# Shadowfear36/SegHiero

Hardware: AMD Instinct MI355X
Metric: images/sec at 512x512 (ResNet-50 2-level), full train step (higher is better)
Workload: dtype f32 (convolutions: exact 3-way bf16 split of every fp32 operand, 6 bf16 MFMA products, f32 accumulate; rest plain f32)

## Files before the change

seghiero_amd/csrc/conv_x6p.hip:

```cpp
#include "conv_x6.h"

__device__ __forceinline__ int swz_row(int row) { return ((row >> 2) & 3) ^ (row & 2); }

#ifndef SH_W1
#define SH_W1(AFF, EPI) ((AFF) == 2 ? 2 : 3)
#define SH_W2(AFF, EPI) (((AFF) == 2 || (EPI) == 2) ? 3 : 4)
#endif
#ifndef SH_X6P_PART
#define SH_X6P_PART 0
#endif
#define SH_PART(n) (SH_X6P_PART == 0 || SH_X6P_PART == (n))
int sh_x6p_launch_dgrad(ConvQ& p, hipStream_t st, int force);
int sh_x6p_wgrad_l0b0(ConvQ& p, bool aff, int wgm, int wgn, int splits, hipStream_t st);
int sh_x6p_wgrad_l1b0(ConvQ& p, bool aff, int wgm, int wgn, int splits, hipStream_t st);
int sh_x6p_wgrad_l0b1(ConvQ& p, bool aff, int wgm, int wgn, int splits, hipStream_t st);
int sh_x6p_wgrad_l1b1(ConvQ& p, bool aff, int wgm, int wgn, int splits, hipStream_t st);
static int x6p_mode() { static int v = -2; if (v == -2) { const char* e = getenv("SEGHIERO_X6P"); v = e ? atoi(e) : 1; } return v; }
[[maybe_unused]] static int x6p_ws() { static int v = -2; if (v == -2) { const char* e = getenv("SEGHIERO_X6P_WS"); v = e ? atoi(e) : 0; } return v; }
static int x6p_tile() { static int v = -2; if (v == -2) { const char* e = getenv("SEGHIERO_X6P_TILE"); v = e ? atoi(e) : 0; } return v; }
#if SH_PART(1) || SH_PART(2) || defined(SH_X6P_EXP)
template <int MODE, int TM, int TN, int WGM, int WGN, int WPS, int AFF, int EPI, int SK, int TAP, int GRP = 0, int ABF = 0, int WS = 0>
__global__ __launch_bounds__(64 * WGM * WGN * (WS ? 2 : 1), WPS) void conv_x6p_kernel(const ConvQ p) {
    constexpr int NT = 64 * WGM * WGN;
    constexpr int BM = 32 * TM * WGM, BN = 32 * TN * WGN;
    constexpr int A_PLANE = BM * ROWB, B_PLANE = BN * ROWB;
    constexpr int RPP = NT / 4;
    constexpr int NA = BM / RPP, NB = BN / RPP;
    static_assert(BM % RPP == 0 && BN % RPP == 0 && RPP % 64 == 0, "tile / thread-count mismatch");
    extern __shared__ __attribute__((aligned(16))) unsigned char smem[];
    unsigned char* const As = smem;
    unsigned char* const Bs = smem + 3 * A_PLANE;
    float* const coef = reinterpret_cast<float*>(smem + 3 * (A_PLANE + B_PLANE));
    static_assert(AFF != 2 || (MODE == DGRAD && TAP == 0 && !GRP), "the deferred BatchNorm-backward loader exists for 1x1 dgrads");
    static_assert(!ABF || (MODE == FPROP && !GRP) || AFF == 2, "bf16 loader streams: the fprop input, or the y stream of the lin loader");
    constexpr bool A_BF = ABF && MODE == FPROP, A2_BF = ABF && AFF == 2;
    constexpr bool A3 = A_BF && AFF == 0;
    auto load_a4 = [&](const __amdgpu_buffer_rsrc_t& rs, unsigned elem_off, unsigned ok, bool bf) -> f32x4 {
        if (bf) {
            const unsigned voff = ((elem_off * 2u) & ok) | (0x80000000u & ~ok);
            const u32x2 r = __builtin_bit_cast(u32x2, __builtin_amdgcn_raw_buffer_load_b64(rs, voff, 0, 0));
            return f32x4{__uint_as_float(r[0]), __uint_as_float(r[1]), 0.f, 0.f};
        }
        const unsigned voff = ((elem_off * 4u) & ok) | (0x80000000u & ~ok);
        return __builtin_bit_cast(f32x4, __builtin_amdgcn_raw_buffer_load_b128(rs, voff, 0, 0));
    };
    auto widen_a4 = [&](f32x4 v, bool bf) -> f32x4 {
        return bf ? bf16x4_to_f32(sh_u32x2{__float_as_uint(v[0]), __float_as_uint(v[1])}) : v;
    };

    const int t_all = threadIdx.x, t = WS ? (t_all & (NT - 1)) : t_all, lane = t & 63, wave = t >> 6;
    [[maybe_unused]] const bool producer = WS && t_all >= NT;
    static_assert(!WS || (NT & (NT - 1)) == 0, "wave-specialised form: power-of-two wave count");
    const int wm = wave / WGN, wn = wave % WGN, l31 = lane & 31, h = lane >> 5;
    const unsigned nblk = (unsigned)p.tiles_m * (unsigned)p.tiles_n;
    const unsigned bid = xcd_remap(blockIdx.x, nblk);
    const int tile_n = bid % p.tiles_n, tile_m = bid / p.tiles_n;
    const int m0 = tile_m * BM, n0 = tile_n * BN;
    const int grp = GRP ? n0 / p.group_n : 0;
    const float* const a_ptr = GRP ? p.ga[grp] : p.a;
    const float* const b_ptr = GRP ? p.gb[grp] : p.b;
    const unsigned a_bytes = GRP ? p.ga_bytes[grp] : p.a_bytes;
    const int lda = (int)(GRP ? p.glda[grp] : p.lda);
    const float* const sc_ptr = GRP ? p.gsc[grp] : p.aff_scale;
    const float* const sh_ptr = GRP ? p.gsh[grp] : p.aff_shift;
    const float aff_floor = (GRP && sc_ptr == nullptr) ? -INFINITY : 0.f;
    int cy = 0, cx = 0, Hc = p.H, Wc = p.W, oy0 = 0, ox0 = 0, ntw = p.KW, Mc = p.M, Kt = p.K;
    if constexpr (MODE == DGRAD) {
        if (p.parity) {
            cy = blockIdx.y >> 1; cx = blockIdx.y & 1;
            oy0 = (cy + p.pad) & 1; ox0 = (cx + p.pad) & 1;
            Hc = (p.H - oy0 + 1) >> 1; Wc = (p.W - ox0 + 1) >> 1;
            const int nth = (p.KH - cy + 1) >> 1;
            ntw = (p.KW - cx + 1) >> 1;
            Mc = p.N * Hc * Wc; Kt = nth * ntw * p.Kc;
            if (m0 >= Mc) return;
        }
    }
    int q_begin = 0, q_end = (Kt + 15) >> 4;
    if constexpr (SK) {
        const int per = ((q_end + p.ksplit - 1) / p.ksplit + 1) & ~1;
        q_begin = min(q_end, (int)blockIdx.y * per); q_end = min(q_end, q_begin + per);
    }
    const int klim = min(Kt, 16 * q_end);
    const int nq = (q_end - q_begin + 1) & ~1;
    constexpr bool single_tap = TAP == 0, tap_uniform = TAP <= 1;

    const __amdgpu_buffer_rsrc_t rsrc_a = __builtin_amdgcn_make_buffer_rsrc(const_cast<float*>(a_ptr), 0, a_bytes, 0x00020000);
    const __amdgpu_buffer_rsrc_t rsrc_b = __builtin_amdgcn_make_buffer_rsrc(const_cast<float*>(b_ptr), 0, p.b_bytes, 0x00020000);
    [[maybe_unused]] const __amdgpu_buffer_rsrc_t rsrc_a2 =
        __builtin_amdgcn_make_buffer_rsrc(const_cast<float*>(AFF == 2 ? p.a2 : a_ptr), 0, AFF == 2 ? p.a2_bytes : a_bytes, 0x00020000);
    constexpr unsigned OOB = 0x80000000u;
    const int kc = t & 3, r0 = t >> 2;
    int a_y[NA], a_x[NA], a_nb[NA];
    int b_row[NB];
    unsigned b_ok[NB];
    int cur_tap = -1;
    const bool direct = TAP == 0 && p.stride == 1 && p.pad == 0 && !(MODE == DGRAD && (p.parity || p.scatter));
#pragma unroll
    for (int i = 0; i < NA; ++i) {
        const int m = m0 + r0 + RPP * i;
        if (direct) { a_y[i] = m < Mc ? 0 : -(1 << 28); a_x[i] = 0; a_nb[i] = m < Mc ? m : 0; }
        else if (m < Mc) {
            if constexpr (MODE == FPROP) {
                const int ow = m % p.Wo, q = m / p.Wo, oh = q % p.Ho, n = q / p.Ho;
                a_y[i] = oh * p.stride - p.pad; a_x[i] = ow * p.stride - p.pad; a_nb[i] = n * p.H * p.W;
            } else {
                const int iwc = m % Wc, q = m / Wc, ihc = q % Hc, n = q / Hc;
                const int ih = p.parity ? 2 * ihc + oy0 : ihc, iw = p.parity ? 2 * iwc + ox0 : iwc;
                a_y[i] = ih + p.pad; a_x[i] = iw + p.pad; a_nb[i] = n * p.Ho * p.Wo;
            }
        } else { a_y[i] = -(1 << 28); a_x[i] = 0; a_nb[i] = 0; }
    }
#pragma unroll
    for (int i = 0; i < NB; ++i) {
        const int j = n0 + r0 + RPP * i;
        b_ok[i] = j < p.Nn ? ~0u : 0u;
        b_row[i] = (GRP ? j - grp * p.group_n : j) * (MODE == FPROP ? p.K : p.Kc);
    }
    int a_off[NA];
    [[maybe_unused]] int a_off2[NA];
    unsigned a_ok[NA];
    auto set_tap = [&](int tap) {
        if (direct) {
#pragma unroll
            for (int i = 0; i < NA; ++i) {
                a_ok[i] = a_y[i] == 0 ? ~0u : 0u;
                a_off[i] = a_nb[i] * lda;
                if constexpr (AFF == 2) a_off2[i] = a_nb[i] * (int)p.lda2;
            }
            return;
        }
        int kh, kw;
        if (MODE == DGRAD && p.parity) { const int ty = tap / ntw; kh = cy + 2 * ty; kw = cx + 2 * (tap - ty * ntw); }
        else { kh = tap / p.KW; kw = tap - kh * p.KW; }
        const int dh = kh * p.dil, dw = kw * p.dil;
#pragma unroll
        for (int i = 0; i < NA; ++i) {
            if constexpr (MODE == FPROP) {
                const int ih = a_y[i] + dh, iw = a_x[i] + dw;
                a_ok[i] = ((unsigned)ih < (unsigned)p.H && (unsigned)iw < (unsigned)p.W) ? ~0u : 0u;
                a_off[i] = (a_nb[i] + ih * p.W + iw) * lda;
            } else {
                int th = a_y[i] - dh, tw = a_x[i] - dw;
                bool ok = th >= 0 && tw >= 0;
                if (p.stride > 1) {
                    ok = ok && (th % p.stride == 0) && (tw % p.stride == 0);
                    th /= p.stride; tw /= p.stride;
                }
                a_ok[i] = (ok && th < p.Ho && tw < p.Wo) ? ~0u : 0u;
                a_off[i] = (a_nb[i] + th * p.Wo + tw) * lda;
                if constexpr (AFF == 2) a_off2[i] = (a_nb[i] + th * p.Wo + tw) * (int)p.lda2;
            }
        }
    };
    auto prepare_tap = [&](int q) {
        if constexpr (TAP == 1) {
            const int tap = (16 * q) / p.Kc;
            if (tap != cur_tap) { set_tap(tap); cur_tap = tap; }
        }
    };
    if constexpr (TAP == 0) { set_tap(0); cur_tap = 0; }
    const f32x4 zero4 = {0.f, 0.f, 0.f, 0.f};
    struct Regs { f32x4 a[NA]; f32x4 a2[AFF == 2 ? NA : 1]; f32x4 b[NB]; int cc; unsigned okm; };
    auto load_half = [&](int q, Regs& R) {
        const int kbase = 16 * q, k = kbase + 4 * kc;
        int tap, cc;
        if constexpr (single_tap) { tap = 0; cc = k; }
        else if constexpr (tap_uniform) { tap = cur_tap; cc = k - tap * p.Kc; }
        else { tap = k / p.Kc; cc = k - tap * p.Kc; set_tap(tap); }
        const unsigned kok = (unsigned)((k - klim) >> 31);
        int wtap = tap;
        if (MODE == DGRAD && p.parity) { const int ty = tap / ntw; wtap = (cy + 2 * ty) * p.KW + cx + 2 * (tap - ty * ntw); }
        R.cc = cc; R.okm = 0;
#pragma unroll
        for (int i = 0; i < NA; ++i) {
            const unsigned ok = kok & a_ok[i];
            R.a[i] = load_a4(rsrc_a, (unsigned)(a_off[i] + cc), ok, A_BF);
            if constexpr (AFF == 2) R.a2[i] = load_a4(rsrc_a2, (unsigned)(a_off2[i] + cc), ok, A2_BF);
            if (AFF) R.okm |= ok & (1u << i);
        }
#pragma unroll
        for (int i = 0; i < NB; ++i) {
            int off;
            if constexpr (MODE == FPROP) off = b_row[i] + k;
            else off = wtap * p.Cin * p.Kc + b_row[i] + cc;
            const unsigned okb = kok & b_ok[i];
            const unsigned voff = (((unsigned)off * 4u) & okb) | (OOB & ~okb);
            R.b[i] = __builtin_bit_cast(f32x4, __builtin_amdgcn_raw_buffer_load_b128(rsrc_b, voff, 0, 0));
        }
    };
    const int swz_w = swz_row(r0);
    auto store_half = [&](Regs& R, int hb) {
        const int off0 = r0 * ROWB + ((((2 * hb) | (kc >> 1)) ^ swz_w) << 4) + ((kc & 1) << 3);
        f32x4 sc = zero4, sh = zero4;
        [[maybe_unused]] f32x4 lmu = zero4, ld_ = zero4;
        if constexpr (AFF) { sc = *reinterpret_cast<const f32x4*>(coef + R.cc); sh = *reinterpret_cast<const f32x4*>(coef + p.Kc + R.cc); }
        if constexpr (AFF == 2) { lmu = *reinterpret_cast<const f32x4*>(coef + 2 * p.Kc + R.cc); ld_ = *reinterpret_cast<const f32x4*>(coef + 3 * p.Kc + R.cc); }
#pragma unroll
        for (int i = 0; i < NA; ++i) {
            if constexpr (A3) {
                *reinterpret_cast<u32x2*>(As + off0 + RPP * i * ROWB) = u32x2{__float_as_uint(R.a[i][0]), __float_as_uint(R.a[i][1])};
                continue;
            }
            f32x4 v = widen_a4(R.a[i], A_BF);
            if constexpr (AFF == 2) {
                const bool ok = (R.okm >> i) & 1u;
                const f32x4 y2 = widen_a4(R.a2[i], A2_BF);
#pragma unroll
                for (int e = 0; e < 4; ++e) { const float w = fmaf(y2[e] - lmu[e], sh[e], fmaf(v[e], sc[e], ld_[e])); v[e] = ok ? w : 0.f; }
            } else if constexpr (AFF) {
                const bool ok = (R.okm >> i) & 1u;
#pragma unroll
                for (int e = 0; e < 4; ++e) { const float w = fmaxf(v[e] * sc[e] + sh[e], aff_floor); v[e] = ok ? w : 0.f; }
            }
            u32x2 q1, q2, q3;
            split4(v, q1, q2, q3);
            const int off = off0 + RPP * i * ROWB;
            *reinterpret_cast<u32x2*>(As + off) = q1;
            *reinterpret_cast<u32x2*>(As + A_PLANE + off) = q2;
            *reinterpret_cast<u32x2*>(As + 2 * A_PLANE + off) = q3;
        }
#pragma unroll
        for (int i = 0; i < NB; ++i) {
            u32x2 q1, q2, q3;
#ifdef SH_ABLATE_BSPLIT
            q1[0] = __float_as_uint(R.b[i][0]); q1[1] = __float_as_uint(R.b[i][1]); q2 = q1; q3[0] = __float_as_uint(R.b[i][2]); q3[1] = __float_as_uint(R.b[i][3]);
#else
            split4(R.b[i], q1, q2, q3);
#endif
            const int off = off0 + RPP * i * ROWB;
            *reinterpret_cast<u32x2*>(Bs + off) = q1;
            *reinterpret_cast<u32x2*>(Bs + B_PLANE + off) = q2;
            *reinterpret_cast<u32x2*>(Bs + 2 * B_PLANE + off) = q3;
        }
    };

    f32x16 acc[TM][TN];
#pragma unroll
    for (int i = 0; i < TM; ++i)
#pragma unroll
        for (int j = 0; j < TN; ++j)
#pragma unroll
            for (int r = 0; r < 16; ++r) acc[i][j][r] = 0.f;

    const int arow = wm * 32 * TM + l31, brow = wn * 32 * TN + l31;
    const int swz_r = swz_row(l31);
    auto compute_half = [&](int hb) {
        const int rd = (((2 * hb) | h) ^ swz_r) << 4;
        bf16x8 bfr[TN][3];
#pragma unroll
        for (int j = 0; j < TN; ++j)
#pragma unroll
            for (int pl = 0; pl < 3; ++pl)
                bfr[j][pl] = __builtin_bit_cast(bf16x8, *reinterpret_cast<const u32x4*>(Bs + pl * B_PLANE + (brow + 32 * j) * ROWB + rd));
#pragma unroll
        for (int i = 0; i < TM; ++i) {
            if constexpr (A3) {
                const bf16x8 a0 = __builtin_bit_cast(bf16x8, *reinterpret_cast<const u32x4*>(As + (arow + 32 * i) * ROWB + rd));
#pragma unroll
                for (int j = 0; j < TN; ++j) acc[i][j] = mma3(a0, bfr[j], acc[i][j]);
            } else {
            bf16x8 af[3];
#pragma unroll
            for (int pl = 0; pl < 3; ++pl)
                af[pl] = __builtin_bit_cast(bf16x8, *reinterpret_cast<const u32x4*>(As + pl * A_PLANE + (arow + 32 * i) * ROWB + rd));
#pragma unroll
            for (int j = 0; j < TN; ++j) acc[i][j] = mma6(af, bfr[j], acc[i][j]);
            }
        }
    };

    auto phase_schedule = [&]() {
        constexpr int PA = A3 ? 1 : 3, PP = A3 ? 3 : 6;
        constexpr int NMFMA = TM * TN * PP, NVALU = 30 * ((A3 ? 0 : NA) + NB) + (AFF == 2 ? 16 : 8 * AFF) * NA, NDSW = PA * NA + 3 * NB,
                      NVM = NA + NB + (AFF == 2 ? NA : 0);
        constexpr int VPM = (NVALU + NMFMA - 1) / NMFMA;
        __builtin_amdgcn_sched_group_barrier(0x100, 3 * TN + PA, 0);
#pragma unroll
        for (int g = 0; g < NMFMA; ++g) {
            __builtin_amdgcn_sched_group_barrier(0x008, 1, 0);
            __builtin_amdgcn_sched_group_barrier(0x002, VPM, 0);
            if (g * NDSW / NMFMA != (g + 1) * NDSW / NMFMA) __builtin_amdgcn_sched_group_barrier(0x200, 1, 0);
            if (g * NVM / NMFMA != (g + 1) * NVM / NMFMA) __builtin_amdgcn_sched_group_barrier(0x020, 1, 0);
            if (g % (PP * TN) == 2 && g / (PP * TN) + 1 < TM) __builtin_amdgcn_sched_group_barrier(0x100, PA, 0);
        }
    };
    if constexpr (AFF == 2) {
        for (int c = t_all; c < 4 * p.Kc; c += NT * (WS ? 2 : 1)) coef[c] = p.lin[c];
        __syncthreads();
    } else if constexpr (AFF) {
        for (int c = t_all; c < p.Kc; c += NT * (WS ? 2 : 1)) { coef[c] = sc_ptr ? sc_ptr[c] : 1.f; coef[p.Kc + c] = sh_ptr ? sh_ptr[c] : 0.f; }
        __syncthreads();
    }
    if constexpr (WS) {
        if (producer) {
            Regs R0, R1;
            prepare_tap(q_begin);     load_half(q_begin, R0);
            prepare_tap(q_begin + 1); load_half(q_begin + 1, R1);
            store_half(R0, 0);
            prepare_tap(q_begin + 2); load_half(q_begin + 2, R0);
            __syncthreads();
            for (int j = 0; j < nq; j += 2) {
                prepare_tap(q_begin + j + 3);
                store_half(R1, 1);
                load_half(q_begin + j + 3, R1);
                __syncthreads();
                prepare_tap(q_begin + j + 4);
                store_half(R0, 0);
                load_half(q_begin + j + 4, R0);
                __syncthreads();
            }
            return;
        }
        __syncthreads();
        for (int j = 0; j < nq; j += 2) {
            compute_half(0);
            __syncthreads();
            compute_half(1);
            __syncthreads();
        }
    } else {
    Regs R0, R1;
    prepare_tap(q_begin);     load_half(q_begin, R0);
    prepare_tap(q_begin + 1); load_half(q_begin + 1, R1);
    store_half(R0, 0);
    prepare_tap(q_begin + 2); load_half(q_begin + 2, R0);
    __syncthreads();
    for (int j = 0; j < nq; j += 2) {
        prepare_tap(q_begin + j + 3);
        store_half(R1, 1);
        load_half(q_begin + j + 3, R1);
        compute_half(0);
        phase_schedule();
        __syncthreads();
        prepare_tap(q_begin + j + 4);
        store_half(R0, 0);
        load_half(q_begin + j + 4, R0);
        compute_half(1);
        phase_schedule();
        __syncthreads();
    }
    }

    if constexpr (SK) {
        float* slab = p.slab + (long long)blockIdx.y * p.M * p.ldslab;
#pragma unroll
        for (int j = 0; j < TN; ++j) {
            const int n = n0 + wn * 32 * TN + 32 * j + l31;
#pragma unroll
            for (int i = 0; i < TM; ++i)
#pragma unroll
                for (int r = 0; r < 16; ++r) {
                    const int m = m0 + wm * 32 * TM + 32 * i + (r & 3) + 8 * (r >> 2) + 4 * h;
                    if (m < p.M && n < p.Nn) slab[(long long)m * p.ldslab + n] = acc[i][j][r];
                }
        }
        return;
    }

    static_assert(EPI == 0 || TM % 2 == 0, "statistics epilogues need whole 64-row groups per wave");
    int ncol[TN];
    bool nok[TN];
    float bias[TN];
    [[maybe_unused]] float b_mu[TN], b_is[TN], b_sc[TN], b_sh[TN];
#pragma unroll
    for (int j = 0; j < TN; ++j) {
        ncol[j] = n0 + wn * 32 * TN + 32 * j + l31;
        nok[j] = ncol[j] < p.Nn;
        bias[j] = (MODE == FPROP && p.extra != nullptr && nok[j]) ? p.extra[ncol[j]] : 0.f;
        if constexpr (EPI == 2) {
            b_mu[j] = b_is[j] = b_sc[j] = b_sh[j] = 0.f;
            if (nok[j]) { b_mu[j] = p.bnb_mean[ncol[j]]; b_is[j] = p.bnb_invstd[ncol[j]]; b_sc[j] = p.bnb_scale[ncol[j]]; b_sh[j] = p.bnb_shift[ncol[j]]; }
        }
    }
    if (EPI == 2 || p.vec_epi) {
        constexpr int WC = 32 * TN, RS = WC + 4, LPR = WC / 4, RPI = 64 / LPR, NRD = 32 / RPI;
        float* const stage = reinterpret_cast<float*>(smem) + wave * (32 * RS);
        const int rr = lane / LPR, c4 = (lane % LPR) * 4;
        const int ncv = n0 + wn * WC + c4;
        const bool nokv = ncv < p.Nn;
        f32x4 vb = zero4, v_mu = zero4, v_is = zero4, v_sc = zero4, v_sh = zero4;
        if (MODE == FPROP && p.extra != nullptr && nokv) vb = ld4(p.extra + ncv);
        if constexpr (EPI == 2) { if (nokv) { v_mu = ld4(p.bnb_mean + ncv); v_is = ld4(p.bnb_invstd + ncv); v_sc = ld4(p.bnb_scale + ncv); v_sh = ld4(p.bnb_shift + ncv); } }
        [[maybe_unused]] f32x4 pend_gs = zero4, pend_gq = zero4;
#pragma unroll
        for (int i = 0; i < TM; ++i) {
#pragma unroll
            for (int j = 0; j < TN; ++j)
#pragma unroll
                for (int r = 0; r < 16; ++r) stage[((r & 3) + 8 * (r >> 2) + 4 * h) * RS + 32 * j + l31] = acc[i][j][r];
            constexpr int CH = (EPI == 2 && NRD > 4) ? 4 : NRD;
            [[maybe_unused]] f32x4 gs = zero4, gq = zero4;
#pragma unroll
            for (int k0 = 0; k0 < NRD; k0 += CH) {
            f32x4 v[CH];
            [[maybe_unused]] f32x4 ad[CH], yv[CH], ov[CH];
            long long mrow[CH];
#pragma unroll
            for (int kk = 0; kk < CH; ++kk) {
                const int row = (k0 + kk) * RPI + rr;
                mrow[kk] = m0 + wm * 32 * TM + 32 * i + row;
                v[kk] = *reinterpret_cast<const f32x4*>(stage + row * RS + c4);
                if constexpr (MODE == DGRAD) {
                    ad[kk] = zero4;
                    if (mrow[kk] < Mc && nokv) {
                        if (p.extra != nullptr) ad[kk] = ld4(p.extra + mrow[kk] * p.ldadd + ncv);
                        if constexpr (EPI == 2) {
                            yv[kk] = lda4(p.bnb_y, mrow[kk] * p.bnb_ldy + ncv, p.act & 4);
                            if (p.bnb_out != nullptr)
                                ov[kk] = (p.act & 64) ? quad_mask_load(p.bnb_out, mrow[kk] * p.bnb_ldo + (ncv >> 2)) : lda4(p.bnb_out, mrow[kk] * p.bnb_ldo + ncv, p.act & 8);
                        }
                    }
                }
            }
#pragma unroll
            for (int kk = 0; kk < CH; ++kk) {
                if (mrow[kk] < Mc && nokv) {
                    f32x4 o = v[kk];
                    if constexpr (MODE == FPROP) o += vb;
                    else {
                        o += ad[kk];
                        if constexpr (EPI == 2) {
                            if (p.bnb_relu) {
                                const f32x4 a = p.bnb_out != nullptr ? ov[kk] : yv[kk] * v_sc + v_sh;
#pragma unroll
                                for (int e = 0; e < 4; ++e) if (!(a[e] > 0.f)) o[e] = 0.f;
                            }
                            gs += o; gq += o * ((yv[kk] - v_mu) * v_is);
                        }
                    }
                    sta4(p.c, mrow[kk] * p.ldc + ncv, o, MODE == FPROP ? (p.act & 2) : 0);
                }
            }
            }
            if constexpr (EPI == 2) {
#pragma unroll
                for (int e = 0; e < 4; ++e) {
#pragma unroll
                    for (int o2 = LPR; o2 < 64; o2 <<= 1) { gs[e] += __shfl_xor(gs[e], o2, 64); gq[e] += __shfl_xor(gq[e], o2, 64); }
                }
                if ((i & 1) == 0) { pend_gs = gs; pend_gq = gq; }
                else {
                    const int pidx = tile_m * (BM / 64) + wm * (TM / 2) + (i >> 1);
                    if (lane < LPR && pidx < p.n_partials && nokv) {
                        st4(p.partials + ((long long)pidx * 2 + 0) * p.Nn + ncv, pend_gs + gs);
                        st4(p.partials + ((long long)pidx * 2 + 1) * p.Nn + ncv, pend_gq + gq);
                    }
                }
            }
        }
    } else if constexpr (EPI != 2) {
    [[maybe_unused]] float pend_s[TN], pend_q[TN];
#pragma unroll
    for (int i = 0; i < TM; ++i) {
        [[maybe_unused]] float gs[TN], gq[TN];
#pragma unroll
        for (int j = 0; j < TN; ++j) { gs[j] = 0.f; gq[j] = 0.f; }
        long long orow[16];
        bool mok[16];
        [[maybe_unused]] float ad[16][TN], yv[16][TN];
#pragma unroll
        for (int r = 0; r < 16; ++r) {
            const int m = m0 + wm * 32 * TM + 32 * i + (r & 3) + 8 * (r >> 2) + 4 * h;
            mok[r] = m < Mc;
            orow[r] = m;
            if constexpr (MODE == DGRAD) {
                if (p.parity) {
                    const int iwc = m % Wc, q2 = m / Wc, ihc = q2 % Hc, nb2 = q2 / Hc;
                    orow[r] = ((long long)nb2 * p.H + 2 * ihc + oy0) * p.W + 2 * iwc + ox0;
                } else if (p.scatter) {
                    const int ow = m % p.W, q = m / p.W, oh = q % p.H, nb = q / p.H;
                    orow[r] = (long long)(nb * p.sH + oh * p.sstride) * p.sW + ow * p.sstride;
                }
#pragma unroll
                for (int j = 0; j < TN; ++j) {
                    ad[r][j] = 0.f;
                    if (mok[r] && nok[j]) {
                        if (p.scatter) ad[r][j] = p.c[orow[r] * p.ldc + ncol[j]];
                        else if (p.extra != nullptr) ad[r][j] = p.extra[orow[r] * p.ldadd + ncol[j]];
                        if constexpr (EPI == 2) yv[r][j] = p.bnb_y[orow[r] * p.bnb_ldy + ncol[j]];
                    }
                }
            }
        }
#pragma unroll
        for (int r = 0; r < 16; ++r) {
#pragma unroll
            for (int j = 0; j < TN; ++j) {
                if (mok[r] && nok[j]) {
                    float v = acc[i][j][r];
                    float* dst = p.c + orow[r] * p.ldc + ncol[j];
                    if constexpr (MODE == FPROP) {
                        *dst = v + bias[j];
                    } else {
                        v += ad[r][j];
                        if constexpr (EPI == 2) {
                            if (p.bnb_relu && !(yv[r][j] * b_sc[j] + b_sh[j] > 0.f)) v = 0.f;
                            gs[j] += v; gq[j] += v * ((yv[r][j] - b_mu[j]) * b_is[j]);
                        }
                        *dst = v;
                    }
                }
            }
        }
        if constexpr (EPI == 2) {
#pragma unroll
            for (int j = 0; j < TN; ++j) {
                const float s1 = gs[j] + __shfl_xor(gs[j], 32, 64), q1 = gq[j] + __shfl_xor(gq[j], 32, 64);
                if ((i & 1) == 0) { pend_s[j] = s1; pend_q[j] = q1; }
                else {
                    const int pidx = tile_m * (BM / 64) + wm * (TM / 2) + (i >> 1);
                    if (h == 0 && pidx < p.n_partials && nok[j]) {
                        p.partials[((long long)pidx * 2 + 0) * p.Nn + ncol[j]] = pend_s[j] + s1;
                        p.partials[((long long)pidx * 2 + 1) * p.Nn + ncol[j]] = pend_q[j] + q1;
                    }
                }
            }
        }
    }
    }
    if constexpr (MODE == FPROP && EPI == 1) {
        if (p.partials != nullptr) {
            const int wrow0 = m0 + wm * 32 * TM;
#pragma unroll
            for (int pr = 0; pr < TM / 2; ++pr) {
                const int prow0 = wrow0 + 64 * pr;
                const int npr = max(0, min(64, p.M - prow0));
                const int pidx = tile_m * (BM / 64) + wm * (TM / 2) + pr;
#pragma unroll
                for (int j = 0; j < TN; ++j) {
                    float ss = 0.f;
#pragma unroll
                    for (int i = 2 * pr; i < 2 * pr + 2; ++i)
#pragma unroll
                        for (int r = 0; r < 16; ++r) ss += acc[i][j][r];
                    ss += __shfl_xor(ss, 32, 64);
                    const float mean = npr > 0 ? ss / (float)npr : 0.f;
                    float qq = 0.f;
#pragma unroll
                    for (int i = 2 * pr; i < 2 * pr + 2; ++i)
#pragma unroll
                        for (int r = 0; r < 16; ++r) {
                            const int row = wrow0 + 32 * i + (r & 3) + 8 * (r >> 2) + 4 * h;
                            const float dv = acc[i][j][r] - mean;
                            qq += (npr == 64 || row < p.M) ? dv * dv : 0.f;
                        }
                    qq += __shfl_xor(qq, 32, 64);
                    const int n = n0 + wn * 32 * TN + 32 * j + l31;
                    if (h == 0 && pidx < p.n_partials && n < p.Nn) {
                        p.partials[((long long)pidx * 2 + 0) * p.Nn + n] = ss;
                        p.partials[((long long)pidx * 2 + 1) * p.Nn + n] = qq;
                    }
                }
            }
        }
    }
}

template <int MODE, int TM, int TN, int WGM, int WGN, int WPS, int AFF, int EPI, int SK, int TAP, int GRP = 0, int ABF = 0, int WS = 0>
static int launch_x6p(ConvQ& p, hipStream_t st) {
    constexpr int BM = 32 * TM * WGM, BN = 32 * TN * WGN;
    const size_t lds = 3 * (size_t)(BM + BN) * ROWB + (AFF == 2 ? 16 : AFF ? 8 : 0) * (size_t)p.Kc;
    if (lds > 160 * 1024) return SH_X6P_NO;
    static size_t attr_lds = 0;
    if (lds > attr_lds) {
        (void)hipFuncSetAttribute(reinterpret_cast<const void*>(&conv_x6p_kernel<MODE, TM, TN, WGM, WGN, WPS, AFF, EPI, SK, TAP, GRP, ABF, WS>),
                                  hipFuncAttributeMaxDynamicSharedMemorySize, (int)(160 * 1024));
        attr_lds = 160 * 1024;
    }
    p.tiles_m = (int)sh_cdiv(p.M, BM);
    p.tiles_n = (int)sh_cdiv(p.Nn, BN);
    dim3 grid((unsigned)(p.tiles_m * p.tiles_n), p.parity ? 4u : (SK ? (unsigned)p.ksplit : 1u));
    conv_x6p_kernel<MODE, TM, TN, WGM, WGN, WPS, AFF, EPI, SK, TAP, GRP, ABF, WS><<<grid, 64 * WGM * WGN * (WS ? 2 : 1), lds, st>>>(p);
    return sh_launch_status();
}

template <int MODE, int AFF, int EPI, int TAP, int ABF = 0>
static int pick_tile_x6p(ConvQ& p, hipStream_t st, int force) {
    (void)force;
    constexpr int W1 = SH_W1(AFF, EPI), W2 = SH_W2(AFF, EPI);
#ifdef SH_X6P_WS
    if (p.Nn > 64 && x6p_ws()) return launch_x6p<MODE, 2, 2, 2, 2, 2, AFF, EPI, 0, TAP, 0, ABF, 1>(p, st);
#endif
    if (p.Nn > 64) return launch_x6p<MODE, 2, 2, 2, 2, W1, AFF, EPI, 0, TAP, 0, ABF>(p, st);
    return launch_x6p<MODE, 2, 1, 2, 2, W2, AFF, EPI, 0, TAP, 0, ABF>(p, st);
}

template <int MODE, int AFF, int EPI, int ABF = 0>
static int pick_x6p(ConvQ& p, hipStream_t st, int force) {
    if constexpr (AFF == 2) {
        if (p.KH * p.KW != 1) return SH_X6P_NO;
        if (p.ksplit > 1) {
            const int rc = launch_x6p<MODE, 2, 2, 2, 2, 2, 2, 0, 1, 0, 0, ABF>(p, st);
            return rc == SH_OK ? sh_x6_splitk_reduce(p, MODE, st) : rc;
        }
        return pick_tile_x6p<MODE, 2, EPI, 0, ABF>(p, st, force);
    } else {
    if (p.ksplit > 1) {
        int rc;
        if (p.KH * p.KW == 1) rc = launch_x6p<MODE, 2, 2, 2, 2, 3, AFF, 0, 1, 0, 0, ABF>(p, st);
        else if ((p.Kc & 15) == 0) rc = launch_x6p<MODE, 2, 2, 2, 2, 3, AFF, 0, 1, 1, 0, ABF>(p, st);
        else return SH_X6P_NO;
        return rc == SH_OK ? sh_x6_splitk_reduce(p, MODE, st) : rc;
    }
    if (p.KH * p.KW == 1) return pick_tile_x6p<MODE, AFF, EPI, 0, ABF>(p, st, force);
    if ((p.Kc & 15) == 0) return pick_tile_x6p<MODE, AFF, EPI, 1, ABF>(p, st, force);
    if (AFF || EPI == 2 || ABF) return SH_X6P_NO;
    return pick_tile_x6p<MODE, 0, EPI, 2>(p, st, force);
    }
}

#endif
#if SH_PART(1)

int sh_x6p_grouped_launch(ConvQ& p, hipStream_t st) {
    if (p.ngroups < 1 || p.ngroups > 6 || (p.group_n & 127) || p.KH * p.KW != 1) return SH_X6P_NO;
    auto al16 = [](const void* q) { return ((uintptr_t)q & 15) == 0; };
    p.vec_epi = (p.ldc & 3) == 0 && al16(p.c);
    return launch_x6p<FPROP, 2, 2, 2, 2, 3, 1, 1, 0, 0, 1>(p, st);
}

int sh_x6p_launch(int mode, ConvQ& p, hipStream_t st) {
    const bool aff = p.aff_scale != nullptr, bnb = p.bnb_y != nullptr;
    if (!x6p_mode() && !aff && !bnb && !p.lin) return SH_X6P_NO;
    const int force = x6p_tile();
    auto al16 = [](const void* q) { return ((uintptr_t)q & 15) == 0; };
    p.vec_epi = !p.parity && !p.scatter && (p.Nn & 3) == 0 && (p.ldc & 3) == 0 && al16(p.c) &&
                (p.extra == nullptr || (al16(p.extra) && (mode == FPROP || (p.ldadd & 3) == 0))) &&
                (!bnb || ((p.bnb_ldy & 3) == 0 && al16(p.bnb_y) && (p.bnb_out == nullptr || (p.act & 64) || ((p.bnb_ldo & 3) == 0 && al16(p.bnb_out))) && al16(p.bnb_mean) && al16(p.bnb_invstd) && al16(p.bnb_scale) &&
                          al16(p.bnb_shift) && al16(p.partials)));
    if (bnb && !p.vec_epi) return SH_X6P_NO;
    { static int v = -2; if (v == -2) { const char* e = getenv("SEGHIERO_X6P_VEC"); v = e ? atoi(e) : 1; } if (!v && !bnb) p.vec_epi = 0; }
    if ((p.act & 2) && !p.vec_epi) return SH_X6P_NO;
    if (mode == FPROP) {
        if (bnb) return SH_EINVAL;
        if (p.act & 1) return aff ? pick_x6p<FPROP, 1, 1, 1>(p, st, force) : pick_x6p<FPROP, 0, 1, 1>(p, st, force);
        if (aff) return pick_x6p<FPROP, 1, 1>(p, st, force);
        return pick_x6p<FPROP, 0, 1>(p, st, force);
    }
    if (aff) return SH_EINVAL;
    return sh_x6p_launch_dgrad(p, st, force);
}
#endif
#if SH_PART(2)
int sh_x6p_launch_dgrad(ConvQ& p, hipStream_t st, int force) {
    const bool bnb = p.bnb_y != nullptr;
    if (p.lin != nullptr && (p.act & 16)) return bnb ? pick_x6p<DGRAD, 2, 2, 1>(p, st, force) : pick_x6p<DGRAD, 2, 0, 1>(p, st, force);
    if (p.lin != nullptr) return bnb ? pick_x6p<DGRAD, 2, 2>(p, st, force) : pick_x6p<DGRAD, 2, 0>(p, st, force);
    if (bnb) return pick_x6p<DGRAD, 0, 2>(p, st, force);
    return pick_x6p<DGRAD, 0, 0>(p, st, force);
}
#endif

#if SH_X6P_PART == 0 || SH_X6P_PART >= 3
template <int WGM, int WGN, int AFF, int LIN = 0, int XBF = 0>
__global__ __launch_bounds__(64 * WGM * WGN, 2) void conv_wgrad_x6p_kernel(const ConvQ p) {
    constexpr int NT = 64 * WGM * WGN, BM = 64 * WGM, BN = 64 * WGN;
    constexpr bool X3 = XBF && AFF == 0;
    constexpr int AROWB = 2 * BM + 64, BROWB = 2 * BN + 64;
    constexpr int APLANE = 32 * AROWB, BPLANE = 32 * BROWB;
    constexpr int ACPR = BM / 4, BCPR = BN / 4;
    constexpr int AKPP = NT / ACPR, BKPP = NT / BCPR;
    constexpr int NA = 16 / AKPP, NB = 16 / BKPP;
    static_assert(NA >= 1 && NB >= 1, "a loader pass must not straddle the two halves");
    extern __shared__ __attribute__((aligned(16))) unsigned char smem[];
    unsigned char* const As = smem;
    unsigned char* const Bs = smem + 3 * APLANE;
    const int t = threadIdx.x, lane = t & 63, wave = t >> 6;
    const int wm = wave / WGN, wn = wave % WGN, l31 = lane & 31, h = lane >> 5;
    const unsigned nblk = (unsigned)p.tiles_m * (unsigned)p.tiles_n;
    unsigned slice, bid;
    if (p.scatter) { const unsigned kq = blockIdx.x >> 3; slice = (kq / nblk) * 8u + (blockIdx.x & 7u); bid = kq % nblk; }
    else { slice = blockIdx.x / nblk; bid = xcd_remap(blockIdx.x % nblk, nblk); }
    if (slice >= (unsigned)p.ksplit) return;
    const int tile_n = bid % p.tiles_n, tile_m = bid / p.tiles_n;
    const int m0 = tile_m * BM, n0 = tile_n * BN;
    const int kbeg = slice * p.kchunk, kend = min(p.K, kbeg + p.kchunk);
    const int nq = (((kend - kbeg + 15) >> 4) + 1) & ~1;

    const __amdgpu_buffer_rsrc_t rsrc_a = __builtin_amdgcn_make_buffer_rsrc(const_cast<float*>(p.a), 0, p.a_bytes, 0x00020000);
    const __amdgpu_buffer_rsrc_t rsrc_b = __builtin_amdgcn_make_buffer_rsrc(const_cast<float*>(p.b), 0, p.b_bytes, 0x00020000);
    [[maybe_unused]] const __amdgpu_buffer_rsrc_t rsrc_a2 =
        __builtin_amdgcn_make_buffer_rsrc(const_cast<float*>(LIN ? p.a2 : p.a), 0, LIN ? p.a2_bytes : p.a_bytes, 0x00020000);
    constexpr unsigned OOB = 0x80000000u;
    const int arc = t % ACPR, ak0 = t / ACPR;
    const int brc = t % BCPR, bk0 = t / BCPR;
    const int co = m0 + 4 * arc;
    const int nn = n0 + 4 * brc;
    const unsigned a_col_ok = co < p.M ? ~0u : 0u, b_col_ok = nn < p.Nn ? ~0u : 0u;
    const int tap = nn / p.Cin, wg_ci = nn - tap * p.Cin;
    const int kh = tap / p.KW, kw = tap - kh * p.KW;
    const int wg_dh = kh * p.dil - p.pad, wg_dw = kw * p.dil - p.pad;
    f32x4 sc = {0.f, 0.f, 0.f, 0.f}, sh = sc;
    if constexpr (AFF) { if (b_col_ok) { sc = ld4(p.aff_scale + wg_ci); sh = ld4(p.aff_shift + wg_ci); } }
    [[maybe_unused]] f32x4 lA = sc, lB = sc, lM = sc, lD = sc;
    if constexpr (LIN) { lA = lB = lM = lD = f32x4{0.f, 0.f, 0.f, 0.f}; if (a_col_ok) { lA = ld4(p.lin + co); lB = ld4(p.lin + p.M + co); lM = ld4(p.lin + 2 * p.M + co); lD = ld4(p.lin + 3 * p.M + co); } }
    int px_ow[NB], px_oh[NB], px_n[NB];
#pragma unroll
    for (int i = 0; i < NB; ++i) {
        const int pix = kbeg + bk0 + BKPP * i;
        px_ow[i] = pix % p.Wo; const int q2 = pix / p.Wo; px_oh[i] = q2 % p.Ho; px_n[i] = q2 / p.Ho;
    }
    auto wg_load4 = [&](const __amdgpu_buffer_rsrc_t& rs, unsigned elem_off, unsigned ok, bool bf) -> f32x4 {
        if (bf) {
            const unsigned voff = ((elem_off * 2u) & ok) | (OOB & ~ok);
            const u32x2 r = __builtin_bit_cast(u32x2, __builtin_amdgcn_raw_buffer_load_b64(rs, voff, 0, 0));
            return f32x4{__uint_as_float(r[0]), __uint_as_float(r[1]), 0.f, 0.f};
        }
        const unsigned voff = ((elem_off * 4u) & ok) | (OOB & ~ok);
        return __builtin_bit_cast(f32x4, __builtin_amdgcn_raw_buffer_load_b128(rs, voff, 0, 0));
    };
    auto wg_widen = [&](f32x4 v, bool bf) -> f32x4 { return bf ? bf16x4_to_f32(sh_u32x2{__float_as_uint(v[0]), __float_as_uint(v[1])}) : v; };
    struct Regs { f32x4 a[NA]; f32x4 a2[LIN ? NA : 1]; f32x4 b[NB]; unsigned okm, okl; };
    auto load_half = [&](int q, Regs& R) {
        const int kbase = kbeg + 16 * q;
        R.okm = 0; R.okl = 0;
#pragma unroll
        for (int i = 0; i < NA; ++i) {
            const int pix = kbase + ak0 + AKPP * i;
            const unsigned ok = (unsigned)((pix - kend) >> 31) & a_col_ok;
            const unsigned voff = (((unsigned)(pix * (int)p.lda + co) * 4u) & ok) | (OOB & ~ok);
            R.a[i] = __builtin_bit_cast(f32x4, __builtin_amdgcn_raw_buffer_load_b128(rsrc_a, voff, 0, 0));
            if constexpr (LIN) {
                R.a2[i] = wg_load4(rsrc_a2, (unsigned)(pix * (int)p.lda2 + co), ok, XBF);
                R.okl |= ok & (1u << i);
            }
        }
#pragma unroll
        for (int i = 0; i < NB; ++i) {
            const int pix = kbase + bk0 + BKPP * i;
            const int ih = px_oh[i] * p.stride + wg_dh, iw = px_ow[i] * p.stride + wg_dw;
            const unsigned inimg = ((unsigned)ih < (unsigned)p.H && (unsigned)iw < (unsigned)p.W) ? ~0u : 0u;
            const unsigned ok = (unsigned)((pix - kend) >> 31) & b_col_ok & inimg;
            R.b[i] = wg_load4(rsrc_b, (unsigned)(((px_n[i] * p.H + ih) * p.W + iw) * (int)p.ldb + wg_ci), ok, XBF);
            if (AFF) R.okm |= ok & (1u << i);
            int ow = px_ow[i] + 16, oh = px_oh[i], n = px_n[i];
            const bool c1 = ow >= p.Wo; ow -= c1 ? p.Wo : 0; oh += c1 ? 1 : 0;
            const bool c2 = oh >= p.Ho; oh -= c2 ? p.Ho : 0; n += c2 ? 1 : 0;
            px_ow[i] = ow; px_oh[i] = oh; px_n[i] = n;
        }
    };
    auto store_half = [&](Regs& R, int hb) {
#pragma unroll
        for (int i = 0; i < NA; ++i) {
            const int off = (16 * hb + ak0 + AKPP * i) * AROWB + arc * 8;
            u32x2 q1, q2, q3;
            f32x4 va = R.a[i];
            if constexpr (LIN) {
                const bool ok = (R.okl >> i) & 1u;
                const f32x4 y2 = wg_widen(R.a2[i], XBF);
#pragma unroll
                for (int e = 0; e < 4; ++e) { const float w = fmaf(y2[e] - lM[e], lB[e], fmaf(va[e], lA[e], lD[e])); va[e] = ok ? w : 0.f; }
            }
            split4(va, q1, q2, q3);
            *reinterpret_cast<u32x2*>(As + off) = q1;
            *reinterpret_cast<u32x2*>(As + APLANE + off) = q2;
            *reinterpret_cast<u32x2*>(As + 2 * APLANE + off) = q3;
        }
#pragma unroll
        for (int i = 0; i < NB; ++i) {
            if constexpr (X3) {
                *reinterpret_cast<u32x2*>(Bs + (16 * hb + bk0 + BKPP * i) * BROWB + brc * 8) = u32x2{__float_as_uint(R.b[i][0]), __float_as_uint(R.b[i][1])};
                continue;
            }
            f32x4 v = wg_widen(R.b[i], XBF);
            if constexpr (AFF) {
                const bool ok = (R.okm >> i) & 1u;
#pragma unroll
                for (int e = 0; e < 4; ++e) { const float w = fmaxf(v[e] * sc[e] + sh[e], 0.f); v[e] = ok ? w : 0.f; }
            }
            const int off = (16 * hb + bk0 + BKPP * i) * BROWB + brc * 8;
            u32x2 q1, q2, q3;
            split4(v, q1, q2, q3);
            *reinterpret_cast<u32x2*>(Bs + off) = q1;
            *reinterpret_cast<u32x2*>(Bs + BPLANE + off) = q2;
            *reinterpret_cast<u32x2*>(Bs + 2 * BPLANE + off) = q3;
        }
    };
    f32x16 acc[2][2];
#pragma unroll
    for (int i = 0; i < 2; ++i)
#pragma unroll
        for (int j = 0; j < 2; ++j)
#pragma unroll
            for (int r = 0; r < 16; ++r) acc[i][j][r] = 0.f;
    const int g = lane >> 4, li = lane & 15, qq = li >> 2, pp = li & 3;
    const int krow = (g >> 1) * 8 + qq, coff = (16 * (g & 1) + 4 * pp) * 2;
    auto frag = [&](const unsigned char* plane, int rowb, int hb, int rowbase) -> bf16x8 {
        const unsigned char* a0 = plane + (krow + hb * 16) * rowb + coff + rowbase * 2;
        const s16x4 v0 = __builtin_amdgcn_ds_read_tr16_b64_v4i16((s16x4 __attribute__((address_space(3)))*)(a0));
        const s16x4 v1 = __builtin_amdgcn_ds_read_tr16_b64_v4i16((s16x4 __attribute__((address_space(3)))*)(a0 + 4 * rowb));
        s16x8 r;
        r[0] = v0[0]; r[1] = v0[1]; r[2] = v0[2]; r[3] = v0[3]; r[4] = v1[0]; r[5] = v1[1]; r[6] = v1[2]; r[7] = v1[3];
        return __builtin_bit_cast(bf16x8, r);
    };
    auto compute_half = [&](int hb) {
        bf16x8 af[2][3], bfr[2][X3 ? 1 : 3];
#pragma unroll
        for (int i = 0; i < 2; ++i)
#pragma unroll
            for (int pl = 0; pl < 3; ++pl) {
                af[i][pl] = frag(As + pl * APLANE, AROWB, hb, wm * 64 + 32 * i);
                if (!X3 || pl == 0) bfr[i][X3 ? 0 : pl] = frag(Bs + pl * BPLANE, BROWB, hb, wn * 64 + 32 * i);
            }
#pragma unroll
        for (int i = 0; i < 2; ++i)
#pragma unroll
            for (int j = 0; j < 2; ++j) {
                if constexpr (X3) acc[i][j] = mma3b(af[i], bfr[j][0], acc[i][j]);
                else acc[i][j] = mma6(af[i], bfr[j], acc[i][j]);
            }
    };
    auto phase_schedule = [&]() {
        constexpr int NMF = X3 ? 12 : 24, NDSR = X3 ? 8 : 12;
        constexpr int NVALU = (X3 ? 2 : 30 + 8 * AFF) * NB + (30 + 16 * LIN) * NA + 8 * NB, NDSW = 3 * NA + (X3 ? 1 : 3) * NB, NVM = NA + NB + LIN * NA;
        constexpr int VPM = (NVALU + NMF - 1) / NMF;
        __builtin_amdgcn_sched_group_barrier(0x100, NDSR, 0);
#pragma unroll
        for (int gq = 0; gq < NMF; ++gq) {
            __builtin_amdgcn_sched_group_barrier(0x008, 1, 0);
            __builtin_amdgcn_sched_group_barrier(0x002, VPM, 0);
            if (gq * NDSW / NMF != (gq + 1) * NDSW / NMF) __builtin_amdgcn_sched_group_barrier(0x200, 1, 0);
            if (gq * NVM / NMF != (gq + 1) * NVM / NMF) __builtin_amdgcn_sched_group_barrier(0x020, 1, 0);
            if (gq == 2) __builtin_amdgcn_sched_group_barrier(0x100, NDSR, 0);
        }
    };
    Regs R0, R1;
    load_half(0, R0);
    load_half(1, R1);
    store_half(R0, 0);
    load_half(2, R0);
    __syncthreads();
    for (int j = 0; j < nq; j += 2) {
        store_half(R1, 1);
        load_half(j + 3, R1);
        compute_half(0);
        phase_schedule();
        __syncthreads();
        store_half(R0, 0);
        load_half(j + 4, R0);
        compute_half(1);
        phase_schedule();
        __syncthreads();
    }
    float* slab = p.c + (long long)slice * p.M * p.Nn;
#pragma unroll
    for (int i = 0; i < 2; ++i)
#pragma unroll
        for (int j = 0; j < 2; ++j) {
            const int n = n0 + wn * 64 + 32 * j + l31;
#pragma unroll
            for (int r = 0; r < 16; ++r) {
                const int m = m0 + wm * 64 + 32 * i + (r & 3) + 8 * (r >> 2) + 4 * h;
                if (m < p.M && n < p.Nn) slab[(long long)m * p.Nn + n] = acc[i][j][r];
            }
        }
}
template <int WGM, int WGN, int AFF, int LIN = 0, int XBF = 0>
static int launch_wgrad_x6p(ConvQ& p, int splits, hipStream_t st) {
    constexpr size_t lds = 3 * 32 * (size_t)((2 * 64 * WGM + 64) + (2 * 64 * WGN + 64));
    static bool attr_done = false;
    if (!attr_done) {
        (void)hipFuncSetAttribute(reinterpret_cast<const void*>(&conv_wgrad_x6p_kernel<WGM, WGN, AFF, LIN, XBF>), hipFuncAttributeMaxDynamicSharedMemorySize, (int)lds);
        attr_done = true;
    }
    p.tiles_m = (int)sh_cdiv(p.M, 64 * WGM); p.tiles_n = (int)sh_cdiv(p.Nn, 64 * WGN);
    p.ksplit = splits;
    const unsigned grid = (unsigned)(p.tiles_m * p.tiles_n) * (unsigned)(p.scatter ? sh_cdiv(splits, 8) * 8 : splits);
    conv_wgrad_x6p_kernel<WGM, WGN, AFF, LIN, XBF><<<grid, 64 * WGM * WGN, lds, st>>>(p);
    return sh_launch_status();
}
template <int AFF, int LIN = 0, int XBF = 0>
static int pick_wgrad_x6p(ConvQ& p, int wgm, int wgn, int splits, hipStream_t st) {
    if (wgm == 4 && wgn == 1) return launch_wgrad_x6p<4, 1, AFF, LIN, XBF>(p, splits, st);
    if (wgm == 2 && wgn == 1) return launch_wgrad_x6p<2, 1, AFF, LIN, XBF>(p, splits, st);
    if (wgm == 2 && wgn == 4) return launch_wgrad_x6p<2, 4, AFF, LIN, XBF>(p, splits, st);
    if (wgm == 1 && wgn == 4) return launch_wgrad_x6p<1, 4, AFF, LIN, XBF>(p, splits, st);
    if (wgm == 1 && wgn == 2) return launch_wgrad_x6p<1, 2, AFF, LIN, XBF>(p, splits, st);
    return launch_wgrad_x6p<2, 2, AFF, LIN, XBF>(p, splits, st);
}
#if SH_PART(3)
int sh_x6p_wgrad_l0b0(ConvQ& p, bool aff, int wgm, int wgn, int splits, hipStream_t st) {
    return aff ? pick_wgrad_x6p<1>(p, wgm, wgn, splits, st) : pick_wgrad_x6p<0>(p, wgm, wgn, splits, st);
}
int sh_x6p_wgrad_launch(ConvQ& p, int wgm, int wgn, int splits, hipStream_t st) {
    const bool aff = p.aff_scale != nullptr;
    if (!x6p_mode() && !aff && !p.lin) return SH_X6P_NO;
    if (p.Wo < 16 || (p.Cin & 3)) return SH_X6P_NO;
    if (p.act & 32) {
        if (p.lin != nullptr && !(p.act & 16)) return SH_X6P_NO;
        return p.lin != nullptr ? sh_x6p_wgrad_l1b1(p, aff, wgm, wgn, splits, st) : sh_x6p_wgrad_l0b1(p, aff, wgm, wgn, splits, st);
    }
    if (p.lin != nullptr && (p.act & 16)) return SH_X6P_NO;
    return p.lin != nullptr ? sh_x6p_wgrad_l1b0(p, aff, wgm, wgn, splits, st) : sh_x6p_wgrad_l0b0(p, aff, wgm, wgn, splits, st);
}
#endif
#if SH_PART(4)
int sh_x6p_wgrad_l1b0(ConvQ& p, bool aff, int wgm, int wgn, int splits, hipStream_t st) {
    return aff ? pick_wgrad_x6p<1, 1>(p, wgm, wgn, splits, st) : pick_wgrad_x6p<0, 1>(p, wgm, wgn, splits, st);
}
#endif
#if SH_PART(5)
int sh_x6p_wgrad_l0b1(ConvQ& p, bool aff, int wgm, int wgn, int splits, hipStream_t st) {
    return aff ? pick_wgrad_x6p<1, 0, 1>(p, wgm, wgn, splits, st) : pick_wgrad_x6p<0, 0, 1>(p, wgm, wgn, splits, st);
}
#endif
#if SH_PART(6)
int sh_x6p_wgrad_l1b1(ConvQ& p, bool aff, int wgm, int wgn, int splits, hipStream_t st) {
    return aff ? pick_wgrad_x6p<1, 1, 1>(p, wgm, wgn, splits, st) : pick_wgrad_x6p<0, 1, 1>(p, wgm, wgn, splits, st);
}
#endif
#endif

#ifdef SH_X6P_EXP
template __global__ void conv_x6p_kernel<SH_X6P_EXP>(const ConvQ);
#endif
```

Measured before the change: 501.3.

## Prefetch BatchNorm-backward epilogue inputs during the dgrad main loop

Adds a dedicated epilogue path for the fused BatchNorm-backward dgrad kernel. It issues the buffer loads of the forward activation y and the ReLU mask a few iterations before the main K loop ends, so their latency overlaps with MFMA work. It also loads the residual-add strips one row group ahead inside the epilogue. The occupancy hints for EPI==2 are lowered to 2 waves per SIMD to make room for the extra prefetch registers, with a fallback to 3 for very large grids. The costs are higher register pressure and lower occupancy, which could hurt the main loop.

```diff
diff --git a/seghiero_amd/csrc/conv_x6p.hip b/seghiero_amd/csrc/conv_x6p.hip
--- a/seghiero_amd/csrc/conv_x6p.hip
+++ b/seghiero_amd/csrc/conv_x6p.hip
@@ -3,9 +3,11 @@
 __device__ __forceinline__ int swz_row(int row) { return ((row >> 2) & 3) ^ (row & 2); }
 
 #ifndef SH_W1
-#define SH_W1(AFF, EPI) ((AFF) == 2 ? 2 : 3)
-#define SH_W2(AFF, EPI) (((AFF) == 2 || (EPI) == 2) ? 3 : 4)
-#endif
+#define SH_W1(AFF, EPI) (((AFF) == 2 || (EPI) == 2) ? 2 : 3)
+#define SH_W2(AFF, EPI) ((EPI) == 2 ? 2 : (AFF) == 2 ? 3 : 4)
+#endif
+#define SH_BNB_PRE_TILES 4096
+#define SH_BNB_LEAD 4
 #ifndef SH_X6P_PART
 #define SH_X6P_PART 0
 #endif
@@ -285,6 +287,57 @@
             if (g % (PP * TN) == 2 && g / (PP * TN) + 1 < TM) __builtin_amdgcn_sched_group_barrier(0x100, PA, 0);
         }
     };
+    constexpr bool PRE = EPI == 2 && WPS <= 2 && (AFF != 2 || TN == 1);
+    static_assert(!PRE || (MODE == DGRAD && !SK && !WS), "the BatchNorm-backward epilogue belongs to the one-pass dgrad");
+    constexpr int E_WC = 32 * TN, E_LPR = E_WC / 4, E_RPI = 64 / E_LPR, E_NRD = 32 / E_RPI;
+    [[maybe_unused]] auto e_pos = [&](int& rr, int& cc) {
+        int tt = t;
+        asm volatile("" : "+v"(tt));
+        const int ln = tt & 63, wv = tt >> 6;
+        rr = (wv / WGN) * 32 * TM + ln / E_LPR; cc = (wv % WGN) * E_WC + (ln % E_LPR) * 4;
+    };
+    constexpr bool E_QM = AFF != 2;
+    [[maybe_unused]] f32x4 ypre[PRE ? TM : 1][PRE ? E_NRD : 1];
+    [[maybe_unused]] unsigned mpre[PRE ? E_NRD : 1];
+    [[maybe_unused]] auto prefetch_bnb = [&]() {
+        int e_rr, e_cc;
+        e_pos(e_rr, e_cc);
+        auto e_ok = [&](int i, int k) -> unsigned { return (m0 + e_rr + 32 * i + k * E_RPI < Mc && n0 + e_cc < p.Nn) ? ~0u : 0u; };
+        const int ybf = (p.act & 4) ? 1 : 0;
+        const __amdgpu_buffer_rsrc_t rs_y = __builtin_amdgcn_make_buffer_rsrc(
+            const_cast<char*>(reinterpret_cast<const char*>(p.bnb_y)) + ((long long)m0 * p.bnb_ldy + n0) * (ybf ? 2 : 4), 0, OOB, 0x00020000);
+        const int ldy = (int)p.bnb_ldy;
+        if (ybf) {
+#pragma unroll
+            for (int i = 0; i < (PRE ? TM : 0); ++i)
+#pragma unroll
+                for (int k = 0; k < E_NRD; ++k) {
+                    const unsigned ok = e_ok(i, k);
+                    const unsigned voff = ((unsigned)(((e_rr + 32 * i + k * E_RPI) * ldy + e_cc) * 2) & ok) | (OOB & ~ok);
+                    const u32x2 r = __builtin_bit_cast(u32x2, __builtin_amdgcn_raw_buffer_load_b64(rs_y, voff, 0, 0));
+                    ypre[i][k] = f32x4{__uint_as_float(r[0]), __uint_as_float(r[1]), 0.f, 0.f};
+                }
+        } else {
+#pragma unroll
+            for (int i = 0; i < (PRE ? TM : 0); ++i)
+#pragma unroll
+                for (int k = 0; k < E_NRD; ++k) {
+                    const unsigned ok = e_ok(i, k);
+                    const unsigned voff = ((unsigned)(((e_rr + 32 * i + k * E_RPI) * ldy + e_cc) * 4) & ok) | (OOB & ~ok);
+                    ypre[i][k] = __builtin_bit_cast(f32x4, __builtin_amdgcn_raw_buffer_load_b128(rs_y, voff, 0, 0));
+                }
+        }
+        if constexpr (!E_QM) return;
+        const bool qm = p.bnb_relu && p.bnb_out != nullptr && (p.act & 64);
+        const __amdgpu_buffer_rsrc_t rs_m = __builtin_amdgcn_make_buffer_rsrc(
+            const_cast<char*>(reinterpret_cast<const char*>(qm ? p.bnb_out : p.bnb_y)) + (qm ? (long long)m0 * p.bnb_ldo + (n0 >> 2) : 0), 0, OOB, 0x00020000);
+#pragma unroll
+        for (int k = 0; k < (PRE ? E_NRD : 0); ++k) {
+            const unsigned ok = qm ? e_ok(0, k) : 0u;
+            const unsigned voff = ((unsigned)((e_rr + k * E_RPI) * (int)p.bnb_ldo + (e_cc >> 2)) & ok) | (OOB & ~ok);
+            mpre[k] = __builtin_amdgcn_raw_buffer_load_b8(rs_m, voff, 0, 0);
+        }
+    };
     if constexpr (AFF == 2) {
         for (int c = t_all; c < 4 * p.Kc; c += NT * (WS ? 2 : 1)) coef[c] = p.lin[c];
         __syncthreads();
@@ -325,8 +378,14 @@
     prepare_tap(q_begin + 1); load_half(q_begin + 1, R1);
     store_half(R0, 0);
     prepare_tap(q_begin + 2); load_half(q_begin + 2, R0);
+    [[maybe_unused]] int jpre = -1;
+    if constexpr (PRE) {
+        jpre = nq - SH_BNB_LEAD;
+        if (jpre <= 0) { prefetch_bnb(); jpre = -1; }
+    }
     __syncthreads();
     for (int j = 0; j < nq; j += 2) {
+        if constexpr (PRE) { if (j == jpre) prefetch_bnb(); }
         prepare_tap(q_begin + j + 3);
         store_half(R1, 1);
         load_half(q_begin + j + 3, R1);
@@ -373,7 +432,97 @@
             if (nok[j]) { b_mu[j] = p.bnb_mean[ncol[j]]; b_is[j] = p.bnb_invstd[ncol[j]]; b_sc[j] = p.bnb_scale[ncol[j]]; b_sh[j] = p.bnb_shift[ncol[j]]; }
         }
     }
-    if (EPI == 2 || p.vec_epi) {
+    if constexpr (PRE) {
+        constexpr int RS = E_WC + 4;
+        int e_rr, e_cc;
+        e_pos(e_rr, e_cc);
+        const int e_ncv = n0 + e_cc;
+        const bool e_nokv = e_ncv < p.Nn;
+        auto e_ok = [&](int i, int k) -> unsigned { return (m0 + e_rr + 32 * i + k * E_RPI < Mc && e_nokv) ? ~0u : 0u; };
+        float* const stage = reinterpret_cast<float*>(smem) + wave * (32 * RS);
+        f32x4 v_mu = zero4, v_is = zero4, v_sc = zero4, v_sh = zero4;
+        if (e_nokv) { v_mu = ld4(p.bnb_mean + e_ncv); v_is = ld4(p.bnb_invstd + e_ncv); v_sc = ld4(p.bnb_scale + e_ncv); v_sh = ld4(p.bnb_shift + e_ncv); }
+        const int mform = !p.bnb_relu ? 0 : (!E_QM || p.bnb_out == nullptr) ? 1 : (p.act & 64) ? 2 : 3;
+        const bool ybf = (p.act & 4) != 0, has_add = p.extra != nullptr;
+        const int obf = (p.act & 8) ? 1 : 0;
+        const __amdgpu_buffer_rsrc_t rs_c = __builtin_amdgcn_make_buffer_rsrc(reinterpret_cast<char*>(p.c) + ((long long)m0 * p.ldc + n0) * 4, 0, OOB, 0x00020000);
+        const __amdgpu_buffer_rsrc_t rs_ad = __builtin_amdgcn_make_buffer_rsrc(
+            const_cast<char*>(reinterpret_cast<const char*>(has_add ? p.extra : p.c)) + (has_add ? ((long long)m0 * p.ldadd + n0) * 4 : 0), 0, OOB, 0x00020000);
+        const __amdgpu_buffer_rsrc_t rs_o = __builtin_amdgcn_make_buffer_rsrc(
+            const_cast<char*>(reinterpret_cast<const char*>(mform >= 2 ? p.bnb_out : p.c)) +
+                (mform == 2 ? (long long)m0 * p.bnb_ldo + (n0 >> 2) : mform == 3 ? ((long long)m0 * p.bnb_ldo + n0) * (obf ? 2 : 4) : 0), 0, OOB, 0x00020000);
+        const int ldc = (int)p.ldc, ldadd = (int)p.ldadd, ldo = (int)p.bnb_ldo;
+        f32x4 ad[TM][E_NRD];
+        unsigned mk[TM][E_NRD];
+        auto load_strip = [&](int i) {
+#pragma unroll
+            for (int k = 0; k < E_NRD; ++k) {
+                const unsigned ok = has_add ? e_ok(i, k) : 0u;
+                const unsigned voff = ((unsigned)(((e_rr + 32 * i + k * E_RPI) * ldadd + e_cc) * 4) & ok) | (OOB & ~ok);
+                ad[i][k] = __builtin_bit_cast(f32x4, __builtin_amdgcn_raw_buffer_load_b128(rs_ad, voff, 0, 0));
+                if (E_QM && i > 0) {
+                    const unsigned okm = mform == 2 ? e_ok(i, k) : 0u;
+                    const unsigned moff = ((unsigned)((e_rr + 32 * i + k * E_RPI) * ldo + (e_cc >> 2)) & okm) | (OOB & ~okm);
+                    mk[i][k] = __builtin_amdgcn_raw_buffer_load_b8(rs_o, moff, 0, 0);
+                }
+            }
+        };
+#pragma unroll
+        for (int k = 0; k < E_NRD; ++k) { mk[0][k] = E_QM ? mpre[k] : 0u; if (!E_QM) mk[TM - 1][k] = 0u; }
+        load_strip(0);
+        f32x4 pend_gs = zero4, pend_gq = zero4;
+#pragma unroll
+        for (int i = 0; i < TM; ++i) {
+#pragma unroll
+            for (int j = 0; j < TN; ++j)
+#pragma unroll
+                for (int r = 0; r < 16; ++r) stage[((r & 3) + 8 * (r >> 2) + 4 * h) * RS + 32 * j + l31] = acc[i][j][r];
+            if (i + 1 < TM) load_strip(i + 1);
+            if (E_QM && mform == 3) {
+                f32x4 ov[E_NRD];
+#pragma unroll
+                for (int k = 0; k < E_NRD; ++k) {
+                    const unsigned ok = e_ok(i, k);
+                    const unsigned voff = ((unsigned)(((e_rr + 32 * i + k * E_RPI) * ldo + e_cc) * (obf ? 2 : 4)) & ok) | (OOB & ~ok);
+                    if (obf) {
+                        const u32x2 r = __builtin_bit_cast(u32x2, __builtin_amdgcn_raw_buffer_load_b64(rs_o, voff, 0, 0));
+                        ov[k] = bf16x4_to_f32(sh_u32x2{r[0], r[1]});
+                    } else ov[k] = __builtin_bit_cast(f32x4, __builtin_amdgcn_raw_buffer_load_b128(rs_o, voff, 0, 0));
+                }
+#pragma unroll
+                for (int k = 0; k < E_NRD; ++k) mk[i][k] = quad_mask_bits(ov[k]);
+            }
+            f32x4 gs = zero4, gq = zero4;
+#pragma unroll
+            for (int k = 0; k < E_NRD; ++k) {
+                const unsigned ok = e_ok(i, k);
+                f32x4 o = *reinterpret_cast<const f32x4*>(stage + (k * E_RPI + lane / E_LPR) * RS + (lane % E_LPR) * 4);
+                o += ad[i][k];
+                const f32x4 yv = ybf ? bf16x4_to_f32(sh_u32x2{__float_as_uint(ypre[i][k][0]), __float_as_uint(ypre[i][k][1])}) : ypre[i][k];
+                const unsigned keep = mform == 0 ? 15u : mform == 1 ? quad_mask_bits(yv * v_sc + v_sh) : mk[i][k];
+#pragma unroll
+                for (int e = 0; e < 4; ++e) o[e] = ((keep >> e) & 1u) ? o[e] : 0.f;
+                const f32x4 oq = o * ((yv - v_mu) * v_is);
+#pragma unroll
+                for (int e = 0; e < 4; ++e) { gs[e] += ok ? o[e] : 0.f; gq[e] += ok ? oq[e] : 0.f; }
+                const unsigned voff = ((unsigned)(((e_rr + 32 * i + k * E_RPI) * ldc + e_cc) * 4) & ok) | (OOB & ~ok);
+                __builtin_amdgcn_raw_buffer_store_b128(__builtin_bit_cast(u32x4, o), rs_c, voff, 0, 0);
+            }
+#pragma unroll
+            for (int e = 0; e < 4; ++e) {
+#pragma unroll
+                for (int o2 = E_LPR; o2 < 64; o2 <<= 1) { gs[e] += __shfl_xor(gs[e], o2, 64); gq[e] += __shfl_xor(gq[e], o2, 64); }
+            }
+            if ((i & 1) == 0) { pend_gs = gs; pend_gq = gq; }
+            else {
+                const int pidx = tile_m * (BM / 64) + wm * (TM / 2) + (i >> 1);
+                if (lane < E_LPR && pidx < p.n_partials && e_nokv) {
+                    st4(p.partials + ((long long)pidx * 2 + 0) * p.Nn + e_ncv, pend_gs + gs);
+                    st4(p.partials + ((long long)pidx * 2 + 1) * p.Nn + e_ncv, pend_gq + gq);
+                }
+            }
+        }
+    } else if (EPI == 2 || p.vec_epi) {
         constexpr int WC = 32 * TN, RS = WC + 4, LPR = WC / 4, RPI = 64 / LPR, NRD = 32 / RPI;
         float* const stage = reinterpret_cast<float*>(smem) + wave * (32 * RS);
         const int rr = lane / LPR, c4 = (lane % LPR) * 4;
@@ -582,6 +731,9 @@
 #ifdef SH_X6P_WS
     if (p.Nn > 64 && x6p_ws()) return launch_x6p<MODE, 2, 2, 2, 2, 2, AFF, EPI, 0, TAP, 0, ABF, 1>(p, st);
 #endif
+    if constexpr (EPI == 2 && AFF != 2) {
+        if (p.Nn > 64 && sh_cdiv(p.M, 128) * sh_cdiv(p.Nn, 128) > SH_BNB_PRE_TILES) return launch_x6p<MODE, 2, 2, 2, 2, 3, AFF, EPI, 0, TAP, 0, ABF>(p, st);
+    }
     if (p.Nn > 64) return launch_x6p<MODE, 2, 2, 2, 2, W1, AFF, EPI, 0, TAP, 0, ABF>(p, st);
     return launch_x6p<MODE, 2, 1, 2, 2, W2, AFF, EPI, 0, TAP, 0, ABF>(p, st);
 }
```

Result: no change. 504.8, median of 6 (+0.7%).
